# Kamino666/S2VT-video-caption

Measured on AMD Instinct MI355X. Metric: training frames/sec (whole node), higher is better.
Workload: dtype f32; 1 GPU; BASELINE configs[1]: S2VT train step, B=64 per GPU x 1 GPU, 80x4096 feats, hidden=embed=1000, vocab=12000, fp32, Adam; global_batch=64, frames=80, parallelism=dp1

## Files before the change

### s2vt-video-caption_amd/csrc/gemm_x3.hip

```cpp
#include <stdlib.h>

#include <type_traits>

#include "common.h"
#include "kernels.h"

namespace s2vt {

typedef short bf16x8 __attribute__((ext_vector_type(8)));
typedef short bf16x4 __attribute__((ext_vector_type(4)));

constexpr int X_REC = 6144;
constexpr int X_NS = 3;

struct GemmX3Args {
    int M, N, K;
    const unsigned short* A; int64_t lda;
    const unsigned short* B; int64_t ldb;
    float* C; int64_t ldc; RowMap cmap;
    const float* bias;
    int accumulate;
    int ksplit;
    float* slabs;
    int ntm, ntn;
};

__device__ __forceinline__ void quad_transpose4(float& a0, float& a1, float& a2, float& a3, bool odd, bool hi) {
    float s, r;
    s = odd ? a0 : a1; r = __builtin_bit_cast(float, __builtin_amdgcn_mov_dpp(__builtin_bit_cast(int, s), 0xB1, 0xF, 0xF, false));
    a0 = odd ? r : a0; a1 = odd ? a1 : r;
    s = odd ? a2 : a3; r = __builtin_bit_cast(float, __builtin_amdgcn_mov_dpp(__builtin_bit_cast(int, s), 0xB1, 0xF, 0xF, false));
    a2 = odd ? r : a2; a3 = odd ? a3 : r;
    s = hi ? a0 : a2; r = __builtin_bit_cast(float, __builtin_amdgcn_mov_dpp(__builtin_bit_cast(int, s), 0x4E, 0xF, 0xF, false));
    a0 = hi ? r : a0; a2 = hi ? a2 : r;
    s = hi ? a1 : a3; r = __builtin_bit_cast(float, __builtin_amdgcn_mov_dpp(__builtin_bit_cast(int, s), 0x4E, 0xF, 0xF, false));
    a1 = hi ? r : a1; a3 = hi ? a3 : r;
}

template <int MI, bool TT>
__global__ __launch_bounds__(512) void gemm_x3_kernel(GemmX3Args p) {
    constexpr int NRA = MI, TMR = 64 * MI, X_STAGE = (NRA + 4) * X_REC;
    __shared__ __attribute__((aligned(1024))) unsigned char smem[X_NS * X_STAGE];
    const unsigned lbase = (unsigned)(uintptr_t)(__attribute__((address_space(3))) unsigned char*)smem;
    const int tid = threadIdx.x, lane = tid & 63;
    const int wave = __builtin_amdgcn_readfirstlane(tid >> 6);
    const int wm = wave >> 2, wn = wave & 3;
    const int li = lane & 31, lh = lane >> 5;

    const int items = p.ntm * p.ntn;
    const int cpx = (items + 7) >> 3, gx = (int)gridDim.x >> 3;
    const int xcd = blockIdx.x & 7;
    const int q_end = ((xcd + 1) * cpx < items) ? (xcd + 1) * cpx : items;
    int q = xcd * cpx + (int)(blockIdx.x >> 3);
    if (q >= q_end) return;
    const int kbeg = blockIdx.y * p.ksplit;
    const int kend = (kbeg + p.ksplit < p.K) ? kbeg + p.ksplit : p.K;
    const int nk = (kend - kbeg) >> 4;
    auto tile_of = [&](int t, int& m0, int& n0) {
        constexpr int GM = 4;
        const int gsz = GM * p.ntn, grp = t / gsz, first_m = grp * GM;
        const int gm = (p.ntm - first_m < GM) ? (p.ntm - first_m) : GM;
        m0 = (first_m + (t % gsz) % gm) * TMR;
        n0 = ((t % gsz) / gm) * 256;
    };

    const bool loader = wave < NRA + 4;
    auto rsrc_of = [&](int m0, int n0) {
        if constexpr (TT) {
            const bool isA = wave < NRA;
            const unsigned short* base = isA ? p.A : p.B;
            const int64_t ld = isA ? p.lda : p.ldb;
            const int c0 = (isA ? m0 : n0) >> 4;
            const int64_t off = (int64_t)(kbeg >> 6) * 64 * ld + (int64_t)c0 * (X_REC / 2);
            int64_t bytes = ((int64_t)((kend - kbeg) >> 6) * 64 * ld - (int64_t)c0 * (X_REC / 2)) * 2;
            if (bytes > 0xFFFFF000ll) bytes = 0xFFFFF000ll;
            return __builtin_amdgcn_make_buffer_rsrc(const_cast<unsigned short*>(base + off), 0, (int)bytes, 0x00020000);
        }
        const bool isA = wave < NRA;
        const int nrb = ((isA ? p.M : p.N) + 63) >> 6;
        int rb = isA ? (m0 >> 6) + wave : (n0 >> 6) + (wave - NRA);
        rb = rb < nrb ? rb : nrb - 1;
        const unsigned short* base = isA ? p.A : p.B;
        const int64_t ld = isA ? p.lda : p.ldb;
        return __builtin_amdgcn_make_buffer_rsrc(const_cast<unsigned short*>(base + (int64_t)rb * 64 * ld + (int64_t)(kbeg >> 4) * (X_REC / 2)), 0,
                                                 nk * X_REC, 0x00020000);
    };
    const int vlane = TT ? ((lane >> 1) & 1) * X_REC + (lane & 1) * 1024 + (lane >> 2) * 16 : lane * 16;
    const int64_t tt_ld2 = (wave < NRA ? p.lda : p.ldb) * 128;
    const int tt_wq = wave < NRA ? wave : wave - NRA;
#define X3_REQ1(J, R, ST, SLOT)                                                                                           \
    if constexpr (TT) {                                                                                                   \
        __builtin_amdgcn_raw_ptr_buffer_load_lds(R, (__attribute__((address_space(3))) void*)(smem + (SLOT) * X_STAGE + (wave < NRA ? 0 : NRA * X_REC) + \
                                                     ((2 * tt_wq + (J) / 3) * 3 + (J) % 3) * 1024),                       \
                                                 16, vlane, (int)(((ST) >> 2) * tt_ld2) + (2 * tt_wq + (J) / 3) * 2 * X_REC + ((J) % 3) * 2048 + ((ST) & 3) * 256, 0, 0); \
    } else {                                                                                                              \
        __builtin_amdgcn_raw_ptr_buffer_load_lds(R, (__attribute__((address_space(3))) void*)(smem + (SLOT) * X_STAGE + wave * X_REC + (J) * 1024), \
                                                 16, vlane, (ST) * X_REC + (J) * 1024, 0, 0);                             \
    }

    f32x16 acc[MI][2];

    unsigned la[MI];
#pragma unroll
    for (int mi = 0; mi < MI; ++mi) {
        const int x = wm * MI + mi;
        la[mi] = lbase + (unsigned)((x >> 1) * X_REC + (x & 1) * 512 + lh * 1024 + li * 16);
    }
    const unsigned lb = lbase + (unsigned)((NRA + wn) * X_REC + lh * 1024 + li * 16);
    const unsigned tt_lane = (unsigned)((8 * lh + ((li & 15) >> 2)) * 64 + (li >> 4) * 32 + (li & 3) * 8);
    const unsigned lb_t = lbase + tt_lane + (unsigned)(NRA * X_REC + wn * 2 * 3072);
    unsigned lat[MI];
#pragma unroll
    for (int mi = 0; mi < MI; ++mi) lat[mi] = lbase + tt_lane + (unsigned)((wm * MI + mi) * 3072);

    bf16x8 a0p[MI], b0p[2];
    auto stage = [&](int g, auto more_tag, bool more_rt, __amdgpu_buffer_rsrc_t r2, int s2, int nwait, bool deferred) {
        const bool more = decltype(more_tag)::value || more_rt;
        if (deferred) {
#pragma unroll
            for (int mi = 0; mi < MI; ++mi)
#pragma unroll
                for (int ni = 0; ni < 2; ++ni) acc[mi][ni] = __builtin_amdgcn_mfma_f32_32x32x16_bf16(a0p[mi], b0p[ni], acc[mi][ni], 0, 0, 0);
        }
        __builtin_amdgcn_sched_barrier(0);
        if (nwait == 6) asm volatile("s_waitcnt vmcnt(6) lgkmcnt(0)\n\ts_barrier" ::: "memory");
        else if (nwait == 0) asm volatile("s_waitcnt vmcnt(0) lgkmcnt(0)\n\ts_barrier" ::: "memory");
        else asm volatile("s_waitcnt vmcnt(%0) lgkmcnt(0)\n\ts_barrier" ::"n"(6 + 8 * MI) : "memory");
        const int slot = g % X_NS, slot2 = (g + 2) % X_NS;
        const unsigned so = (unsigned)(slot * X_STAGE);
        bf16x8 a[3][MI], b[3][2];
#define X3_RD(DST, ADDR, OFF) asm volatile("ds_read_b128 %0, %1 offset:%2" : "=v"(DST) : "v"(ADDR), "n"(OFF));
#define X3_RDT(DST, ADDR, OFF)                                                                                               \
    {                                                                                                                        \
        bf16x4 lo_, hi_;                                                                                                     \
        asm volatile("ds_read_b64_tr_b16 %0, %1 offset:%2" : "=v"(lo_) : "v"(ADDR), "n"(OFF));                               \
        asm volatile("ds_read_b64_tr_b16 %0, %1 offset:%2" : "=v"(hi_) : "v"(ADDR), "n"((OFF) + 256));                       \
        DST = __builtin_shufflevector(lo_, hi_, 0, 1, 2, 3, 4, 5, 6, 7);                                                     \
    }
#define X3_LDA(PL)                                                                                                           \
    if constexpr (TT) { _Pragma("unroll") for (int mi = 0; mi < MI; ++mi) { X3_RDT(a[PL][mi], lat[mi] + so, (PL) * 1024) } } \
    else { _Pragma("unroll") for (int mi = 0; mi < MI; ++mi) { X3_RD(a[PL][mi], la[mi] + so, (PL) * 2048) } }
#define X3_LDB(PL)                                                                                                           \
    if constexpr (TT) { const unsigned b_ = lb_t + so; X3_RDT(b[PL][0], b_, (PL) * 1024) X3_RDT(b[PL][1], b_, (3 + (PL)) * 1024) } \
    else { const unsigned b_ = lb + so; X3_RD(b[PL][0], b_, (PL) * 2048) X3_RD(b[PL][1], b_, (PL) * 2048 + 512) }
#define X3_WAIT(N, PA, PB)                                                                                     \
    {                                                                                                          \
        asm volatile("s_waitcnt lgkmcnt(%0)" ::"n"(N));                                                        \
        _Pragma("unroll") for (int i_ = 0; i_ < MI; ++i_) asm volatile("" : "+v"(a[PA][i_]));                  \
        asm volatile("" : "+v"(b[PB][0]));                                                                     \
        asm volatile("" : "+v"(b[PB][1]));                                                                     \
    }
        __builtin_amdgcn_sched_barrier(0);
        X3_LDA(1) X3_LDB(1) X3_LDA(0) X3_LDB(2)
        if constexpr (!TT) { X3_LDA(2) X3_LDB(0) }
#define X3_PROD(PA, PB)                                                                                          \
    _Pragma("unroll") for (int mi = 0; mi < MI; ++mi) _Pragma("unroll") for (int ni = 0; ni < 2; ++ni)           \
        acc[mi][ni] = __builtin_amdgcn_mfma_f32_32x32x16_bf16(a[PA][mi], b[PB][ni], acc[mi][ni], 0, 0, 0);
        const bool req = more && loader;
#define X3_GROUP(N, PA, PB, J, DOWAIT)                                     \
    if constexpr (DOWAIT) { X3_WAIT(N, PA, PB) }                           \
    X3_PROD(PA, PB)                                                        \
    if (req) { X3_REQ1(J, r2, s2, slot2) }                                 \
    __builtin_amdgcn_sched_barrier(0);
        if (req) { X3_REQ1(5, r2, s2, slot2) }
        __builtin_amdgcn_sched_barrier(0);
        if constexpr (TT) {
            X3_GROUP(2 * (MI + 2), 1, 1, 0, true)
            X3_LDA(2) X3_LDB(0)
            X3_GROUP(2 * (MI + 2), 0, 2, 1, true)
            X3_GROUP(0, 2, 0, 2, true)
        } else {
            X3_GROUP(2 * (MI + 2), 1, 1, 0, true)
            X3_GROUP(MI + 2, 0, 2, 1, true)
            X3_GROUP(0, 2, 0, 2, true)
        }
        X3_GROUP(0, 0, 1, 3, false)
        X3_GROUP(0, 1, 0, 4, false)
#pragma unroll
        for (int mi = 0; mi < MI; ++mi) a0p[mi] = a[0][mi];
        b0p[0] = b[0][0]; b0p[1] = b[0][1];
#undef X3_GROUP
#undef X3_PROD
#undef X3_WAIT
#undef X3_RD
#undef X3_RDT
#undef X3_LDA
#undef X3_LDB
    };

    int m0, n0;
    tile_of(q, m0, n0);
    __amdgpu_buffer_rsrc_t r0 = rsrc_of(m0, n0);
    if (loader) {
#pragma unroll
        for (int j = 0; j < 6; ++j) { X3_REQ1(j, r0, 0, 0) }
#pragma unroll
        for (int j = 0; j < 6; ++j) { X3_REQ1(j, r0, 1, 1) }
    }
    int s = 0;
    int qn = q + gx;
    int m1 = 0, n1 = 0;
    if (qn < q_end) tile_of(qn, m1, n1);
    __amdgpu_buffer_rsrc_t r1 = rsrc_of(m1, n1);
    int nwait = 6;
#pragma unroll
    for (int mi = 0; mi < MI; ++mi)
#pragma unroll
        for (int ni = 0; ni < 2; ++ni)
#pragma unroll
            for (int r = 0; r < 16; ++r) acc[mi][ni][r] = 0.f;
    for (int g = 0;; ++g) {
        const bool has_next = qn < q_end;
        for (; s + 2 < nk; ++s, ++g) {
            stage(g, std::true_type{}, true, r0, s + 2, nwait, s > 0);
            nwait = 6;
        }
        stage(g, std::false_type{}, has_next, r1, 0, nwait, true);
        ++g;
        stage(g, std::false_type{}, has_next, r1, 1, has_next ? 6 : 0, true);
#pragma unroll
        for (int mi = 0; mi < MI; ++mi)
#pragma unroll
            for (int ni = 0; ni < 2; ++ni) acc[mi][ni] = __builtin_amdgcn_mfma_f32_32x32x16_bf16(a0p[mi], b0p[ni], acc[mi][ni], 0, 0, 0);

        bool counted;
        {
            int e_li = li, e_lh = lh;
            asm volatile("" : "+v"(e_li), "+v"(e_lh));
            const int t = e_li & 3;
            const bool odd = t & 1, hi = t & 2;
            const int ncol = n0 + wn * 64 + (e_li & ~3);
            const bool vec = p.slabs ? ((p.N & 3) == 0 && (reinterpret_cast<uintptr_t>(p.slabs) & 15) == 0)
                                     : ((p.ldc & 3) == 0 && (reinterpret_cast<uintptr_t>(p.C) & 15) == 0);
            counted = m0 + TMR <= p.M && n0 + wn * 64 + 64 <= p.N;
            f32x4 bv[2] = {f32x4{0.f, 0.f, 0.f, 0.f}, f32x4{0.f, 0.f, 0.f, 0.f}};
            if (p.bias && !p.slabs) {
#pragma unroll
                for (int ni = 0; ni < 2; ++ni)
#pragma unroll
                    for (int k = 0; k < 4; ++k) {
                        const int n = ncol + ni * 32 + k;
                        bv[ni][k] = n < p.N ? p.bias[n] : 0.f;
                    }
            }
#pragma unroll
            for (int mi = 0; mi < MI; ++mi) {
                __builtin_amdgcn_sched_barrier(0);
#pragma unroll
                for (int j = 0; j < 4; ++j) {
                    const int m = m0 + wm * 32 * MI + mi * 32 + 8 * j + 4 * e_lh + t;
                    f32x4 v[2];
#pragma unroll
                    for (int ni = 0; ni < 2; ++ni) {
                        float a0 = acc[mi][ni][4 * j], a1 = acc[mi][ni][4 * j + 1], a2 = acc[mi][ni][4 * j + 2], a3 = acc[mi][ni][4 * j + 3];
                        quad_transpose4(a0, a1, a2, a3, odd, hi);
                        v[ni] = f32x4{a0, a1, a2, a3};
                    }
                    if (m >= p.M) continue;
                    float* row = p.slabs ? p.slabs + ((int64_t)blockIdx.y * p.M + m) * p.N : p.C + (int64_t)map_row(p.cmap, m) * p.ldc;
#pragma unroll
                    for (int ni = 0; ni < 2; ++ni) {
                        const int n = ncol + ni * 32;
                        f32x4 o = v[ni];
                        if (!p.slabs) { o[0] += bv[ni][0]; o[1] += bv[ni][1]; o[2] += bv[ni][2]; o[3] += bv[ni][3]; }
                        if (vec && n + 4 <= p.N) {
                            f32x4* q4 = reinterpret_cast<f32x4*>(row + n);
                            if (p.accumulate && !p.slabs) { const f32x4 c = *q4; o[0] += c[0]; o[1] += c[1]; o[2] += c[2]; o[3] += c[3]; }
                            *q4 = o;
                        } else {
#pragma unroll
                            for (int k = 0; k < 4; ++k)
                                if (n + k < p.N) {
                                    float x = o[k];
                                    if (p.accumulate && !p.slabs) x += row[n + k];
                                    row[n + k] = x;
                                }
                        }
                    }
                }
            }
        }
        if (!has_next) break;
        nwait = counted ? 6 + 8 * MI : 6;
        q = qn; m0 = m1; n0 = n1; r0 = r1;
        qn = q + gx;
        if (qn < q_end) tile_of(qn, m1, n1);
        r1 = rsrc_of(m1, n1);
        s = 0;
#pragma unroll
        for (int mi = 0; mi < MI; ++mi)
#pragma unroll
            for (int ni = 0; ni < 2; ++ni)
#pragma unroll
                for (int r = 0; r < 16; ++r) acc[mi][ni][r] = 0.f;
    }
#undef X3_REQ1
}

int splitk_reduce(hipStream_t stream, const float* slabs, int nsplit, int M, int N, float* C, int64_t ldc, RowMap cmap,
                  const float* bias, bool accumulate);

static const double kX3Stage[5] = {0, 0, 1.35, 1.75, 2.15};
static const double kX3Epi[5] = {0, 0, 4.5, 6.0, 8.0};
static int g_x3_force_mi = 0, g_x3_force_n = 0;
void gemm_x3_tune(int tile_rows, int nsplit) {
    g_x3_force_mi = (tile_rows >= 128 && tile_rows <= 256 && tile_rows % 64 == 0) ? tile_rows / 64 : 0;
    g_x3_force_n = nsplit > 0 ? nsplit : 0;
}

static int gemm_x3_impl(hipStream_t stream, bool tt, int M, int N, int K, const unsigned short* A, int64_t lda, const unsigned short* B,
                       int64_t ldb, float* C, int64_t ldc, RowMap cmap, const float* bias, bool accumulate, float* splitk_ws,
                       size_t splitk_ws_floats);
int gemm_x3(hipStream_t stream, int M, int N, int K, const unsigned short* A, int64_t lda, const unsigned short* B,
            int64_t ldb, float* C, int64_t ldc, RowMap cmap, const float* bias, bool accumulate, float* splitk_ws,
            size_t splitk_ws_floats) {
    return gemm_x3_impl(stream, false, M, N, K, A, lda, B, ldb, C, ldc, cmap, bias, accumulate, splitk_ws, splitk_ws_floats);
}
int gemm_x3_tt(hipStream_t stream, int M, int N, int K, const unsigned short* A, int64_t lda, const unsigned short* B,
               int64_t ldb, float* C, int64_t ldc, RowMap cmap, const float* bias, bool accumulate, float* splitk_ws,
               size_t splitk_ws_floats) {
    return gemm_x3_impl(stream, true, M, N, K, A, lda, B, ldb, C, ldc, cmap, bias, accumulate, splitk_ws, splitk_ws_floats);
}
static int gemm_x3_impl(hipStream_t stream, bool tt, int M, int N, int K, const unsigned short* A, int64_t lda, const unsigned short* B,
                       int64_t ldb, float* C, int64_t ldc, RowMap cmap, const float* bias, bool accumulate, float* splitk_ws,
                       size_t splitk_ws_floats) {
    if (M <= 0 || N <= 0) return 0;
    if (tt) {
        S2VT_REQUIRE(K > 0 && K % 64 == 0 && lda % 8 == 0 && ldb % 8 == 0 && lda >= 3 * (int64_t)((M + 63) / 64 * 64) &&
                         ldb >= 3 * (int64_t)((N + 63) / 64 * 64) && (reinterpret_cast<uintptr_t>(A) & 15) == 0 &&
                         (reinterpret_cast<uintptr_t>(B) & 15) == 0,
                     "gemm_x3_tt: K (image rows) must be a multiple of 64, the row images hold pad64(M) / pad64(N) columns");
    } else
    S2VT_REQUIRE(K > 0 && K % 64 == 0 && lda % 8 == 0 && ldb % 8 == 0 && lda >= 3 * (int64_t)K && ldb >= 3 * (int64_t)K &&
                     (reinterpret_cast<uintptr_t>(A) & 15) == 0 && (reinterpret_cast<uintptr_t>(B) & 15) == 0,
                 "gemm_x3: K must be the zero-padded multiple of 64 of the blocked plane layout, operands 16-B aligned");
    GemmX3Args p;
    p.M = M; p.N = N; p.K = K;
    p.A = A; p.lda = lda;
    p.B = B; p.ldb = ldb;
    p.C = C; p.ldc = ldc; p.cmap = cmap; p.bias = bias; p.accumulate = accumulate ? 1 : 0;
    const int ncu = planned_compute_units();
    const int force_mi = g_x3_force_mi, force_n = g_x3_force_n;
    const int ntn = cdiv(N, 256);
    int best_mi = 4, best_ns = 1, best_g = 8;
    double best = 1e30;
    const int64_t ldmax = lda > ldb ? lda : ldb, kTTSpan = 0xFFFFF000ll;
    static const int order[3] = {4, 3, 2};
    for (int oi = 0; oi < 3; ++oi) {
        const int mi = order[oi];
        if (force_mi && force_mi != mi) continue;
        const int tiles = cdiv(M, 64 * mi) * ntn;
        for (int n = 1; n <= 16; ++n) {
            if (n > 1 && (!splitk_ws || K < 512 || K / n < 256 || (size_t)n * M * N > splitk_ws_floats)) break;
            if (force_n && n != force_n) continue;
            const int ks = cdiv(cdiv(K, n), 64) * 64, nn = cdiv(K, ks);
            if (nn != n) continue;
            if (tt && (int64_t)ks * ldmax * 2 >= kTTSpan) continue;
            int g = ncu / nn / 8 * 8;
            if (g < 8) g = 8;
            if (g > cdiv(tiles, 8) * 8) g = cdiv(tiles, 8) * 8;
            const int per_wg = cdiv(cdiv(tiles, 8), g / 8);
            const double rounds = (double)cdiv(g * nn, ncu);
            const double t = rounds * per_wg * ((ks / 16) * kX3Stage[mi] + kX3Epi[mi]) + 3.0 +
                             (nn > 1 ? (nn + 1.0) * M * (double)N * 4.0 / 3.5e6 + 8.0 : 0.0);
            if (t < best * 0.98) { best = t; best_mi = mi; best_ns = nn; best_g = g; }
        }
    }
    if (best > 1e29) {
        S2VT_REQUIRE(!tt || (int64_t)K * ldmax * 2 < kTTSpan,
                     "gemm_x3_tt: a row image of %lld bytes needs k slices below 4 GB and split-K scratch for them (%zu floats given)",
                     (long long)((int64_t)K * ldmax * 2), splitk_ws_floats);
        best_mi = 4; best_ns = 1;
        best_g = cdiv(cdiv(M, 256) * ntn, 8) * 8;
        if (best_g > ncu) best_g = ncu;
    }
    p.ntm = cdiv(M, 64 * best_mi); p.ntn = ntn;
    p.ksplit = (best_ns > 1) ? cdiv(cdiv(K, best_ns), 64) * 64 : K;
    const int nsplit = (best_ns > 1) ? cdiv(K, p.ksplit) : 1;
    p.slabs = (nsplit > 1) ? splitk_ws : nullptr;
    const dim3 grid(best_g, nsplit);
    if (tt) {
        switch (best_mi) {
            case 2: hipLaunchKernelGGL((gemm_x3_kernel<2, true>), grid, dim3(512), 0, stream, p); break;
            case 3: hipLaunchKernelGGL((gemm_x3_kernel<3, true>), grid, dim3(512), 0, stream, p); break;
            default: hipLaunchKernelGGL((gemm_x3_kernel<4, true>), grid, dim3(512), 0, stream, p); break;
        }
    } else {
        switch (best_mi) {
            case 2: hipLaunchKernelGGL((gemm_x3_kernel<2, false>), grid, dim3(512), 0, stream, p); break;
            case 3: hipLaunchKernelGGL((gemm_x3_kernel<3, false>), grid, dim3(512), 0, stream, p); break;
            default: hipLaunchKernelGGL((gemm_x3_kernel<4, false>), grid, dim3(512), 0, stream, p); break;
        }
    }
    S2VT_LAUNCH_CHECK("gemm_x3_kernel");
    if (nsplit > 1) return splitk_reduce(stream, splitk_ws, nsplit, M, N, C, ldc, cmap, bias, accumulate);
    return 0;
}

}
```

Before: 505,300 frames/s.

## Switch gemm_x3 to 16x16x32 MFMA tiles with reorganized LDS fragment schedule

Replaces the 32x32x16 bf16 MFMA accumulators with 16x16x32 MFMA tiles (2*MI by 4 blocks per wave) and rewrites the LDS fragment addressing, the read/compute interleave and the epilogue row/column mapping to match. It also swizzles the per-lane chunk order in the transposed-layout global-to-LDS loads. The intent is to cut LDS read traffic or bank conflicts and improve overlap of ds_reads with MFMA. In exchange, each wave issues more, smaller MFMA instructions, and the new layout is more complex, so it risks higher register pressure and subtle indexing errors.

```diff
diff --git a/s2vt-video-caption_amd/csrc/gemm_x3.hip b/s2vt-video-caption_amd/csrc/gemm_x3.hip
--- a/s2vt-video-caption_amd/csrc/gemm_x3.hip
+++ b/s2vt-video-caption_amd/csrc/gemm_x3.hip
@@ -85,7 +85,8 @@
         return __builtin_amdgcn_make_buffer_rsrc(const_cast<unsigned short*>(base + (int64_t)rb * 64 * ld + (int64_t)(kbeg >> 4) * (X_REC / 2)), 0,
                                                  nk * X_REC, 0x00020000);
     };
-    const int vlane = TT ? ((lane >> 1) & 1) * X_REC + (lane & 1) * 1024 + (lane >> 2) * 16 : lane * 16;
+    const int vchunk = (lane & 3) ^ ((lane >> 4) & 2);
+    const int vlane = TT ? ((vchunk >> 1) & 1) * X_REC + (vchunk & 1) * 1024 + (lane >> 2) * 16 : lane * 16;
     const int64_t tt_ld2 = (wave < NRA ? p.lda : p.ldb) * 128;
     const int tt_wq = wave < NRA ? wave : wave - NRA;
 #define X3_REQ1(J, R, ST, SLOT)                                                                                           \
@@ -98,29 +99,36 @@
                                                  16, vlane, (ST) * X_REC + (J) * 1024, 0, 0);                             \
     }
 
-    f32x16 acc[MI][2];
-
-    unsigned la[MI];
+    f32x4 acc[2 * MI][4];
+
+    const int r16 = lane & 15, gh = (lane >> 4) & 1, gp = lane >> 5;
+    auto kind_nn = [&](int lo, int hi) { return (unsigned)((2 * (gp ? hi : lo) + gh) * 1024 + r16 * 16); };
+    auto kind_tt = [&](int lo, int hi) {
+        return (unsigned)((8 * gh + (r16 >> 2)) * 64 + 32 * gh + (r16 & 3) * 8 + (gp ? hi : lo) * 1024);
+    };
+    unsigned laX[MI], laY[MI], lbU, lbV, lbW;
 #pragma unroll
     for (int mi = 0; mi < MI; ++mi) {
         const int x = wm * MI + mi;
-        la[mi] = lbase + (unsigned)((x >> 1) * X_REC + (x & 1) * 512 + lh * 1024 + li * 16);
-    }
-    const unsigned lb = lbase + (unsigned)((NRA + wn) * X_REC + lh * 1024 + li * 16);
-    const unsigned tt_lane = (unsigned)((8 * lh + ((li & 15) >> 2)) * 64 + (li >> 4) * 32 + (li & 3) * 8);
-    const unsigned lb_t = lbase + tt_lane + (unsigned)(NRA * X_REC + wn * 2 * 3072);
-    unsigned lat[MI];
-#pragma unroll
-    for (int mi = 0; mi < MI; ++mi) lat[mi] = lbase + tt_lane + (unsigned)((wm * MI + mi) * 3072);
-
-    bf16x8 a0p[MI], b0p[2];
+        const unsigned t = lbase + (unsigned)(TT ? x * 3072 : (x >> 1) * X_REC + (x & 1) * 512);
+        laX[mi] = t + (TT ? kind_tt(1, 0) : kind_nn(1, 0));
+        laY[mi] = t + (TT ? kind_tt(2, 0) : kind_nn(2, 0));
+    }
+    {
+        const unsigned t = lbase + (unsigned)(NRA * X_REC + (TT ? wn * 2 * 3072 : wn * X_REC));
+        lbU = t + (TT ? kind_tt(0, 0) : kind_nn(0, 0));
+        lbV = t + (TT ? kind_tt(1, 2) : kind_nn(1, 2));
+        lbW = t + (TT ? kind_tt(0, 1) : kind_nn(0, 1));
+    }
+
+    bf16x8 fx[2 * MI], fu[4];
     auto stage = [&](int g, auto more_tag, bool more_rt, __amdgpu_buffer_rsrc_t r2, int s2, int nwait, bool deferred) {
         const bool more = decltype(more_tag)::value || more_rt;
         if (deferred) {
 #pragma unroll
-            for (int mi = 0; mi < MI; ++mi)
-#pragma unroll
-                for (int ni = 0; ni < 2; ++ni) acc[mi][ni] = __builtin_amdgcn_mfma_f32_32x32x16_bf16(a0p[mi], b0p[ni], acc[mi][ni], 0, 0, 0);
+            for (int u = 0; u < 2 * MI; ++u)
+#pragma unroll
+                for (int v = 0; v < 4; ++v) acc[u][v] = __builtin_amdgcn_mfma_f32_16x16x32_bf16(fx[u], fu[v], acc[u][v], 0, 0, 0);
         }
         __builtin_amdgcn_sched_barrier(0);
         if (nwait == 6) asm volatile("s_waitcnt vmcnt(6) lgkmcnt(0)\n\ts_barrier" ::: "memory");
@@ -128,7 +136,7 @@
         else asm volatile("s_waitcnt vmcnt(%0) lgkmcnt(0)\n\ts_barrier" ::"n"(6 + 8 * MI) : "memory");
         const int slot = g % X_NS, slot2 = (g + 2) % X_NS;
         const unsigned so = (unsigned)(slot * X_STAGE);
-        bf16x8 a[3][MI], b[3][2];
+        bf16x8 fy[2 * MI], fv[4], fw[4];
 #define X3_RD(DST, ADDR, OFF) asm volatile("ds_read_b128 %0, %1 offset:%2" : "=v"(DST) : "v"(ADDR), "n"(OFF));
 #define X3_RDT(DST, ADDR, OFF)                                                                                               \
     {                                                                                                                        \
@@ -137,50 +145,49 @@
         asm volatile("ds_read_b64_tr_b16 %0, %1 offset:%2" : "=v"(hi_) : "v"(ADDR), "n"((OFF) + 256));                       \
         DST = __builtin_shufflevector(lo_, hi_, 0, 1, 2, 3, 4, 5, 6, 7);                                                     \
     }
-#define X3_LDA(PL)                                                                                                           \
-    if constexpr (TT) { _Pragma("unroll") for (int mi = 0; mi < MI; ++mi) { X3_RDT(a[PL][mi], lat[mi] + so, (PL) * 1024) } } \
-    else { _Pragma("unroll") for (int mi = 0; mi < MI; ++mi) { X3_RD(a[PL][mi], la[mi] + so, (PL) * 2048) } }
-#define X3_LDB(PL)                                                                                                           \
-    if constexpr (TT) { const unsigned b_ = lb_t + so; X3_RDT(b[PL][0], b_, (PL) * 1024) X3_RDT(b[PL][1], b_, (3 + (PL)) * 1024) } \
-    else { const unsigned b_ = lb + so; X3_RD(b[PL][0], b_, (PL) * 2048) X3_RD(b[PL][1], b_, (PL) * 2048 + 512) }
-#define X3_WAIT(N, PA, PB)                                                                                     \
+#define X3_LDA(F, BASE)                                                                                                      \
+    _Pragma("unroll") for (int mi = 0; mi < MI; ++mi) {                                                                      \
+        const unsigned a_ = BASE[mi] + so;                                                                                   \
+        if constexpr (TT) { X3_RDT(F[2 * mi], a_, 0) X3_RDT(F[2 * mi + 1], a_ ^ 32u, 0) }                                   \
+        else { X3_RD(F[2 * mi], a_, 0) X3_RD(F[2 * mi + 1], a_, 256) }                                                       \
+    }
+#define X3_LDB(F, BASE)                                                                                                      \
+    {                                                                                                                        \
+        const unsigned b_ = BASE + so;                                                                                       \
+        if constexpr (TT) { X3_RDT(F[0], b_, 0) X3_RDT(F[1], b_ ^ 32u, 0) X3_RDT(F[2], b_, 3072) X3_RDT(F[3], b_ ^ 32u, 3072) } \
+        else { X3_RD(F[0], b_, 0) X3_RD(F[1], b_, 256) X3_RD(F[2], b_, 512) X3_RD(F[3], b_, 768) }                           \
+    }
+#define X3_WAIT(N, FA, FB)                                                                                     \
     {                                                                                                          \
         asm volatile("s_waitcnt lgkmcnt(%0)" ::"n"(N));                                                        \
-        _Pragma("unroll") for (int i_ = 0; i_ < MI; ++i_) asm volatile("" : "+v"(a[PA][i_]));                  \
-        asm volatile("" : "+v"(b[PB][0]));                                                                     \
-        asm volatile("" : "+v"(b[PB][1]));                                                                     \
-    }
+        _Pragma("unroll") for (int i_ = 0; i_ < 2 * MI; ++i_) asm volatile("" : "+v"(FA[i_]));                 \
+        _Pragma("unroll") for (int i_ = 0; i_ < 4; ++i_) asm volatile("" : "+v"(FB[i_]));                      \
+    }
+#define X3_HALF(FA, FB, V0, J)                                                                                   \
+    _Pragma("unroll") for (int u = 0; u < 2 * MI; ++u) _Pragma("unroll") for (int v = V0; v < V0 + 2; ++v)      \
+        acc[u][v] = __builtin_amdgcn_mfma_f32_16x16x32_bf16(FA[u], FB[v], acc[u][v], 0, 0, 0);                   \
+    if (req) { X3_REQ1(J, r2, s2, slot2) }                                                                       \
+    __builtin_amdgcn_sched_barrier(0);
+        const bool req = more && loader;
         __builtin_amdgcn_sched_barrier(0);
-        X3_LDA(1) X3_LDB(1) X3_LDA(0) X3_LDB(2)
-        if constexpr (!TT) { X3_LDA(2) X3_LDB(0) }
-#define X3_PROD(PA, PB)                                                                                          \
-    _Pragma("unroll") for (int mi = 0; mi < MI; ++mi) _Pragma("unroll") for (int ni = 0; ni < 2; ++ni)           \
-        acc[mi][ni] = __builtin_amdgcn_mfma_f32_32x32x16_bf16(a[PA][mi], b[PB][ni], acc[mi][ni], 0, 0, 0);
-        const bool req = more && loader;
-#define X3_GROUP(N, PA, PB, J, DOWAIT)                                     \
-    if constexpr (DOWAIT) { X3_WAIT(N, PA, PB) }                           \
-    X3_PROD(PA, PB)                                                        \
-    if (req) { X3_REQ1(J, r2, s2, slot2) }                                 \
-    __builtin_amdgcn_sched_barrier(0);
+        X3_LDA(fx, laX) X3_LDB(fv, lbV)
+        X3_WAIT(0, fx, fv)
         if (req) { X3_REQ1(5, r2, s2, slot2) }
         __builtin_amdgcn_sched_barrier(0);
-        if constexpr (TT) {
-            X3_GROUP(2 * (MI + 2), 1, 1, 0, true)
-            X3_LDA(2) X3_LDB(0)
-            X3_GROUP(2 * (MI + 2), 0, 2, 1, true)
-            X3_GROUP(0, 2, 0, 2, true)
-        } else {
-            X3_GROUP(2 * (MI + 2), 1, 1, 0, true)
-            X3_GROUP(MI + 2, 0, 2, 1, true)
-            X3_GROUP(0, 2, 0, 2, true)
-        }
-        X3_GROUP(0, 0, 1, 3, false)
-        X3_GROUP(0, 1, 0, 4, false)
-#pragma unroll
-        for (int mi = 0; mi < MI; ++mi) a0p[mi] = a[0][mi];
-        b0p[0] = b[0][0]; b0p[1] = b[0][1];
-#undef X3_GROUP
-#undef X3_PROD
+        X3_HALF(fx, fv, 0, 0)
+        X3_LDA(fy, laY)
+        if constexpr (MI < 4) { X3_LDB(fw, lbW) }
+        X3_HALF(fx, fv, 2, 1)
+        if constexpr (MI == 4) { X3_LDB(fw, lbW) }
+        X3_WAIT(0, fy, fw)
+        X3_HALF(fy, fw, 0, 2)
+        if constexpr (MI == 4) { X3_LDA(fx, laX) }
+        X3_LDB(fu, lbU)
+        X3_HALF(fy, fw, 2, 3)
+        X3_WAIT(0, fx, fu)
+        if (req) { X3_REQ1(4, r2, s2, slot2) }
+        __builtin_amdgcn_sched_barrier(0);
+#undef X3_HALF
 #undef X3_WAIT
 #undef X3_RD
 #undef X3_RDT
@@ -204,11 +211,9 @@
     __amdgpu_buffer_rsrc_t r1 = rsrc_of(m1, n1);
     int nwait = 6;
 #pragma unroll
-    for (int mi = 0; mi < MI; ++mi)
-#pragma unroll
-        for (int ni = 0; ni < 2; ++ni)
-#pragma unroll
-            for (int r = 0; r < 16; ++r) acc[mi][ni][r] = 0.f;
+    for (int u = 0; u < 2 * MI; ++u)
+#pragma unroll
+        for (int v = 0; v < 4; ++v) acc[u][v] = f32x4{0.f, 0.f, 0.f, 0.f};
     for (int g = 0;; ++g) {
         const bool has_next = qn < q_end;
         for (; s + 2 < nk; ++s, ++g) {
@@ -219,63 +224,63 @@
         ++g;
         stage(g, std::false_type{}, has_next, r1, 1, has_next ? 6 : 0, true);
 #pragma unroll
-        for (int mi = 0; mi < MI; ++mi)
-#pragma unroll
-            for (int ni = 0; ni < 2; ++ni) acc[mi][ni] = __builtin_amdgcn_mfma_f32_32x32x16_bf16(a0p[mi], b0p[ni], acc[mi][ni], 0, 0, 0);
+        for (int u = 0; u < 2 * MI; ++u)
+#pragma unroll
+            for (int v = 0; v < 4; ++v) acc[u][v] = __builtin_amdgcn_mfma_f32_16x16x32_bf16(fx[u], fu[v], acc[u][v], 0, 0, 0);
 
         bool counted;
         {
-            int e_li = li, e_lh = lh;
-            asm volatile("" : "+v"(e_li), "+v"(e_lh));
-            const int t = e_li & 3;
+            int e_l = lane;
+            asm volatile("" : "+v"(e_l));
+            const int t = e_l & 3;
             const bool odd = t & 1, hi = t & 2;
-            const int ncol = n0 + wn * 64 + (e_li & ~3);
+            const int ncol = n0 + wn * 64 + (e_l & 12);
+            const int mrow = m0 + wm * 32 * MI + 4 * (e_l >> 4) + t;
             const bool vec = p.slabs ? ((p.N & 3) == 0 && (reinterpret_cast<uintptr_t>(p.slabs) & 15) == 0)
                                      : ((p.ldc & 3) == 0 && (reinterpret_cast<uintptr_t>(p.C) & 15) == 0);
             counted = m0 + TMR <= p.M && n0 + wn * 64 + 64 <= p.N;
-            f32x4 bv[2] = {f32x4{0.f, 0.f, 0.f, 0.f}, f32x4{0.f, 0.f, 0.f, 0.f}};
-            if (p.bias && !p.slabs) {
-#pragma unroll
-                for (int ni = 0; ni < 2; ++ni)
+            f32x4 bv[4];
+#pragma unroll
+            for (int v = 0; v < 4; ++v) {
+                bv[v] = f32x4{0.f, 0.f, 0.f, 0.f};
+                if (p.bias && !p.slabs) {
 #pragma unroll
                     for (int k = 0; k < 4; ++k) {
-                        const int n = ncol + ni * 32 + k;
-                        bv[ni][k] = n < p.N ? p.bias[n] : 0.f;
+                        const int n = ncol + v * 16 + k;
+                        bv[v][k] = n < p.N ? p.bias[n] : 0.f;
                     }
+                }
             }
 #pragma unroll
-            for (int mi = 0; mi < MI; ++mi) {
+            for (int u = 0; u < 2 * MI; ++u) {
                 __builtin_amdgcn_sched_barrier(0);
-#pragma unroll
-                for (int j = 0; j < 4; ++j) {
-                    const int m = m0 + wm * 32 * MI + mi * 32 + 8 * j + 4 * e_lh + t;
-                    f32x4 v[2];
-#pragma unroll
-                    for (int ni = 0; ni < 2; ++ni) {
-                        float a0 = acc[mi][ni][4 * j], a1 = acc[mi][ni][4 * j + 1], a2 = acc[mi][ni][4 * j + 2], a3 = acc[mi][ni][4 * j + 3];
-                        quad_transpose4(a0, a1, a2, a3, odd, hi);
-                        v[ni] = f32x4{a0, a1, a2, a3};
-                    }
-                    if (m >= p.M) continue;
-                    float* row = p.slabs ? p.slabs + ((int64_t)blockIdx.y * p.M + m) * p.N : p.C + (int64_t)map_row(p.cmap, m) * p.ldc;
-#pragma unroll
-                    for (int ni = 0; ni < 2; ++ni) {
-                        const int n = ncol + ni * 32;
-                        f32x4 o = v[ni];
-                        if (!p.slabs) { o[0] += bv[ni][0]; o[1] += bv[ni][1]; o[2] += bv[ni][2]; o[3] += bv[ni][3]; }
-                        if (vec && n + 4 <= p.N) {
-                            f32x4* q4 = reinterpret_cast<f32x4*>(row + n);
-                            if (p.accumulate && !p.slabs) { const f32x4 c = *q4; o[0] += c[0]; o[1] += c[1]; o[2] += c[2]; o[3] += c[3]; }
-                            *q4 = o;
-                        } else {
-#pragma unroll
-                            for (int k = 0; k < 4; ++k)
-                                if (n + k < p.N) {
-                                    float x = o[k];
-                                    if (p.accumulate && !p.slabs) x += row[n + k];
-                                    row[n + k] = x;
-                                }
-                        }
+                const int m = mrow + 16 * u;
+                f32x4 o4[4];
+#pragma unroll
+                for (int v = 0; v < 4; ++v) {
+                    float a0 = acc[u][v][0], a1 = acc[u][v][1], a2 = acc[u][v][2], a3 = acc[u][v][3];
+                    quad_transpose4(a0, a1, a2, a3, odd, hi);
+                    o4[v] = f32x4{a0, a1, a2, a3};
+                }
+                if (m >= p.M) continue;
+                float* row = p.slabs ? p.slabs + ((int64_t)blockIdx.y * p.M + m) * p.N : p.C + (int64_t)map_row(p.cmap, m) * p.ldc;
+#pragma unroll
+                for (int v = 0; v < 4; ++v) {
+                    const int n = ncol + v * 16;
+                    f32x4 o = o4[v];
+                    if (!p.slabs) { o[0] += bv[v][0]; o[1] += bv[v][1]; o[2] += bv[v][2]; o[3] += bv[v][3]; }
+                    if (vec && n + 4 <= p.N) {
+                        f32x4* q4 = reinterpret_cast<f32x4*>(row + n);
+                        if (p.accumulate && !p.slabs) { const f32x4 c = *q4; o[0] += c[0]; o[1] += c[1]; o[2] += c[2]; o[3] += c[3]; }
+                        *q4 = o;
+                    } else {
+#pragma unroll
+                        for (int k = 0; k < 4; ++k)
+                            if (n + k < p.N) {
+                                float x = o[k];
+                                if (p.accumulate && !p.slabs) x += row[n + k];
+                                row[n + k] = x;
+                            }
                     }
                 }
             }
@@ -288,11 +293,9 @@
         r1 = rsrc_of(m1, n1);
         s = 0;
 #pragma unroll
-        for (int mi = 0; mi < MI; ++mi)
-#pragma unroll
-            for (int ni = 0; ni < 2; ++ni)
-#pragma unroll
-                for (int r = 0; r < 16; ++r) acc[mi][ni][r] = 0.f;
+        for (int u = 0; u < 2 * MI; ++u)
+#pragma unroll
+            for (int v = 0; v < 4; ++v) acc[u][v] = f32x4{0.f, 0.f, 0.f, 0.f};
     }
 #undef X3_REQ1
 }
```

Result: faster. 512,600 frames/s, median of 6 (+1.4%).
